# NVIDIA/audio-flamingo

Measured on AMD Instinct MI355X. Metric: audio-sec/s + decoder tokens/s, AF3-7B bf16 train, higher is better.
Workload: dtype bf16; 1 GPU; AF3 (AF-Whisper 32L + Qwen2.5-7B 28L, MLP projector) bf16 train step fwd+bwd+AdamW, 30 s clips, S=1024; micro_batch_per_gpu=8, global_batch=8, seq_len=1024, parallelism=dp1, activation_checkpointing=False

## Files before the change

### audio-flamingo_amd/csrc/common.h

```cpp
#pragma once
#include <hip/hip_runtime.h>
#include <stdint.h>
#include <stdio.h>
#include <stdarg.h>
#include <type_traits>
#include <utility>

typedef __bf16 bf16;
typedef __attribute__((ext_vector_type(2))) __bf16 bf16x2;
typedef __attribute__((ext_vector_type(4))) __bf16 bf16x4;
typedef __attribute__((ext_vector_type(8))) __bf16 bf16x8;
typedef __attribute__((ext_vector_type(2))) float f32x2;
typedef __attribute__((ext_vector_type(4))) float f32x4;
typedef __attribute__((ext_vector_type(16))) float f32x16;

#define AFK_OK 0
#define AFK_ERR_ARG (-1)
#define AFK_ERR_LAUNCH (-2)
#define AFK_ERR_UNSUPPORTED (-3)

int afk_set_error(int code, const char* fmt, ...);
void afk_count(int id);

#define AFK_REQUIRE(cond, ...)                                   \
// ... 80 lines not shown
}

__device__ __forceinline__ float bf2f(bf16 x) { return (float)x; }
__device__ __forceinline__ bf16 f2bf(float x) { return (bf16)x; }
__device__ __forceinline__ float rbf(float x) { return (float)((bf16)x); }
__device__ __forceinline__ float rbf_strict(float x) {
    const bf16 h = (bf16)x;
    return __uint_as_float((uint32_t)__builtin_bit_cast(unsigned short, h) << 16);
}

__device__ __forceinline__ float wave_sum(float v) {
#pragma unroll
    for (int o = 32; o > 0; o >>= 1) v += __shfl_xor(v, o, 64);
    return v;
}
__device__ __forceinline__ float wave_max(float v) {
#pragma unroll
    for (int o = 32; o > 0; o >>= 1) v = fmaxf(v, __shfl_xor(v, o, 64));
    return v;
}

template <int NW>
__device__ __forceinline__ float block_sum(float v, float* scratch) {
    v = wave_sum(v);
    const int lane = threadIdx.x & 63, w = threadIdx.x >> 6;
    __syncthreads();
    if (lane == 0) scratch[w] = v;
    __syncthreads();
    float r = 0.f;
#pragma unroll
    for (int i = 0; i < NW; ++i) r += scratch[i];
    return r;
}
template <int NW>
__device__ __forceinline__ float block_max(float v, float* scratch) {
    v = wave_max(v);
    const int lane = threadIdx.x & 63, w = threadIdx.x >> 6;
    __syncthreads();
    if (lane == 0) scratch[w] = v;
    __syncthreads();
    float r = scratch[0];
#pragma unroll
    for (int i = 1; i < NW; ++i) r = fmaxf(r, scratch[i]);
    return r;
}

__device__ __forceinline__ float sigmoid_f(float x) { return 1.f / (1.f + __expf(-x)); }
__device__ __forceinline__ float gelu_f(float x) { return 0.5f * x * (1.f + erff(x * 0.70710678118654752440f)); }
__device__ __forceinline__ float gelu_grad_f(float x) {
    const float cdf = 0.5f * (1.f + erff(x * 0.70710678118654752440f));
    const float pdf = 0.39894228040143267794f * __expf(-0.5f * x * x);
    return cdf + x * pdf;
}
```

### audio-flamingo_amd/csrc/elementwise.hip

```cpp
#include "common.h"
#include "../../include/afk.h"

namespace {

inline int ew_grid(int64_t n_items, int per_block) {
    int64_t g = afk_cdiv(n_items, per_block);
    if (g > 4096) g = 4096;
    if (g < 1) g = 1;
    return (int)g;
}

__global__ __launch_bounds__(256) void transpose_kernel(const bf16* __restrict__ in0, bf16* __restrict__ out0, int R, int C,
                                                        int Rpad, int64_t ld_in, int64_t ld_out, int nb2,
                                                        int64_t bs1_in, int64_t bs2_in, int64_t bs1_out, int64_t bs2_out,
                                                        int tiles_x, int tiles_y, int64_t ntiles) {
    __shared__ bf16 tile[64][66];
    const int t = threadIdx.x;
    for (int64_t tix = blockIdx.x; tix < ntiles; tix += gridDim.x) {
        const int bx = (int)(tix % tiles_x);
        const int by = (int)((tix / tiles_x) % tiles_y);
        const int b = (int)(tix / ((int64_t)tiles_x * tiles_y));
        const int b1 = b / nb2, b2 = b - b1 * nb2;
        const bf16* in = in0 + b1 * bs1_in + b2 * bs2_in;
        bf16* out = out0 + b1 * bs1_out + b2 * bs2_out;
// ... 94 lines not shown
            const float silu = gf * s;
            og[e] = (bf16)(df * uf * (s * (1.f + gf * (1.f - s))));
            ou[e] = (bf16)(df * silu);
        }
        *(bf16x8*)(dgu + r * 2 * I + c) = og;
        *(bf16x8*)(dgu + r * 2 * I + I + c) = ou;
    }
}

__global__ __launch_bounds__(256) void rope_kernel(bf16* __restrict__ buf, const bf16* __restrict__ cos_t,
                                                   const bf16* __restrict__ sin_t, const int* __restrict__ pos, int64_t rows,
                                                   int S, int ld, int nheads, int D, float sign) {
    const int half = D >> 1, vph = half >> 2;
    const int64_t total = rows * nheads * vph;
    for (int64_t i = (int64_t)blockIdx.x * 256 + threadIdx.x; i < total; i += (int64_t)gridDim.x * 256) {
        const int v = (int)(i % vph);
        const int64_t t = i / vph;
        const int h = (int)(t % nheads);
        const int64_t r = t / nheads;
        const int p = pos ? pos[r] : (int)(r % S);
        bf16* x1p = buf + r * ld + h * D + 4 * v;
        bf16* x2p = x1p + half;
        const bf16x4 x1 = *(const bf16x4*)x1p, x2 = *(const bf16x4*)x2p;
        const bf16x4 c1 = *(const bf16x4*)(cos_t + (int64_t)p * D + 4 * v);
        const bf16x4 s1 = *(const bf16x4*)(sin_t + (int64_t)p * D + 4 * v);
        const bf16x4 c2 = *(const bf16x4*)(cos_t + (int64_t)p * D + half + 4 * v);
        const bf16x4 s2 = *(const bf16x4*)(sin_t + (int64_t)p * D + half + 4 * v);
        bf16x4 o1, o2;
#pragma unroll
        for (int e = 0; e < 4; ++e) {
            const float a = (float)x1[e], b = (float)x2[e];
            o1[e] = (bf16)(rbf_strict(a * (float)c1[e]) + rbf_strict(-sign * b * (float)s1[e]));
            o2[e] = (bf16)(rbf_strict(b * (float)c2[e]) + rbf_strict(sign * a * (float)s2[e]));
        }
        *(bf16x4*)x1p = o1;
        *(bf16x4*)x2p = o2;
    }
}

__global__ __launch_bounds__(256) void add_kernel(const bf16* __restrict__ a, const bf16* __restrict__ b, bf16* __restrict__ o,
                                                  int64_t nvec) {
    for (int64_t i = (int64_t)blockIdx.x * 256 + threadIdx.x; i < nvec; i += (int64_t)gridDim.x * 256) {
        const bf16x8 x = *(const bf16x8*)(a + 8 * i), y = *(const bf16x8*)(b + 8 * i);
        bf16x8 r;
#pragma unroll
        for (int e = 0; e < 8; ++e) r[e] = (bf16)((float)x[e] + (float)y[e]);
        *(bf16x8*)(o + 8 * i) = r;
    }
}

__global__ __launch_bounds__(256) void scale_add_kernel(const bf16* x, bf16* y, int64_t nvec, const float* __restrict__ scale,
                                                        int accumulate) {
    const float a = *scale;
    for (int64_t i = (int64_t)blockIdx.x * 256 + threadIdx.x; i < nvec; i += (int64_t)gridDim.x * 256) {
        const bf16x8 xv = *(const bf16x8*)(x + 8 * i);
        bf16x8 o;
        if (accumulate) {
            const bf16x8 yv = *(const bf16x8*)(y + 8 * i);
#pragma unroll
            for (int e = 0; e < 8; ++e) o[e] = (bf16)((float)yv[e] + a * (float)xv[e]);
        } else {
#pragma unroll
            for (int e = 0; e < 8; ++e) o[e] = (bf16)(a * (float)xv[e]);
        }
        *(bf16x8*)(y + 8 * i) = o;
    }
}

__global__ __launch_bounds__(256) void cast_f32_bf16_kernel(const float* __restrict__ a, bf16* __restrict__ o, int64_t n) {
    for (int64_t i = (int64_t)blockIdx.x * 256 + threadIdx.x; i < n; i += (int64_t)gridDim.x * 256) o[i] = (bf16)a[i];
}

__global__ __launch_bounds__(256) void rowsum_kernel(const bf16* __restrict__ in, int64_t ld, int C, bf16* __restrict__ out,
                                                     int rows, int accumulate) {
    const int lane = threadIdx.x & 63;
    const int row = blockIdx.x * 4 + (threadIdx.x >> 6);
    if (row >= rows) return;
    const bf16* p = in + (int64_t)row * ld;
    float s = 0.f;
    const int nv = C >> 3;
    for (int v = lane; v < nv; v += 64) {
        const bf16x8 t = *(const bf16x8*)(p + 8 * v);
#pragma unroll
        for (int e = 0; e < 8; ++e) s += (float)t[e];
    }
    for (int c = nv * 8 + lane; c < C; c += 64) s += (float)p[c];
    s = wave_sum(s);
    if (lane == 0) out[row] = (bf16)(accumulate ? s + (float)out[row] : s);
}

template <bool FUSED>
__global__ __launch_bounds__(256) void colsum_partial_kernel(const bf16* __restrict__ in, int64_t ld, int64_t rows, int cols,
                                                             float* __restrict__ partial, int rows_per_slice, int* __restrict__ counters,
                                                             bf16* __restrict__ out, int accumulate) {
    __shared__ float red[32][65];
    __shared__ int last_flag;
    const int cl = threadIdx.x & 7, rl = threadIdx.x >> 3;
    const int c0 = blockIdx.x * 64 + cl * 8;
    const int64_t r_begin = (int64_t)blockIdx.y * rows_per_slice;
    const int64_t r_end = min(rows, r_begin + rows_per_slice);
    float acc[8];
#pragma unroll
    for (int e = 0; e < 8; ++e) acc[e] = 0.f;
    if (c0 < cols) {
        for (int64_t r = r_begin + rl; r < r_end; r += 32) {
            const bf16x8 t = *(const bf16x8*)(in + r * ld + c0);
// ... 194 lines not shown
        __syncthreads();
    }
    if (tid == 0) *n_audio = carry;
}

__global__ __launch_bounds__(256) void embed_scatter_fwd_kernel(const int64_t* __restrict__ ids, const int* __restrict__ src,
                                                                const bf16* __restrict__ embed, const bf16* __restrict__ audio,
                                                                bf16* __restrict__ out, int64_t n, int H) {
    const int vpr = H >> 3;
    const int64_t total = n * vpr;
    for (int64_t i = (int64_t)blockIdx.x * 256 + threadIdx.x; i < total; i += (int64_t)gridDim.x * 256) {
        const int v = (int)(i % vpr);
        const int64_t r = i / vpr;
        const int s = src ? src[r] : -1;
        const bf16* p = (s >= 0) ? audio + (int64_t)s * H : embed + ids[r] * H;
        *(bf16x8*)(out + r * H + 8 * v) = *(const bf16x8*)(p + 8 * v);
    }
}

__global__ __launch_bounds__(256) void embed_scatter_bwd_kernel(const int64_t* __restrict__ ids, const int* __restrict__ src,
                                                                const bf16* __restrict__ dout, bf16* __restrict__ d_embed,
                                                                bf16* __restrict__ d_audio, const int* __restrict__ perm, int64_t n, int H) {
    const int vpr = H >> 3;
    const int64_t total = n * vpr;
    for (int64_t i = (int64_t)blockIdx.x * 256 + threadIdx.x; i < total; i += (int64_t)gridDim.x * 256) {
        const int v = (int)(i % vpr);
        const int64_t j = i / vpr;
        const int64_t r = perm ? perm[j] : j;
        const int s = src ? src[r] : -1;
        if (s >= 0) {
            if (d_audio) *(bf16x8*)(d_audio + (int64_t)s * H + 8 * v) = *(const bf16x8*)(dout + r * H + 8 * v);
            continue;
        }
        if (!d_embed) continue;
        const int64_t id = ids[r];
        if (j > 0 && ids[perm[j - 1]] == id) continue;
        float acc[8] = {0.f, 0.f, 0.f, 0.f, 0.f, 0.f, 0.f, 0.f};
        for (int64_t k = j; k < n; ++k) {
            const int64_t rk = perm[k];
            if (ids[rk] != id) break;
            const bf16x8 d = *(const bf16x8*)(dout + rk * H + 8 * v);
#pragma unroll
            for (int e = 0; e < 8; ++e) acc[e] += (float)d[e];
        }
        bf16* p = d_embed + id * H + 8 * v;
        const bf16x8 old = *(const bf16x8*)p;
        bf16x8 o;
#pragma unroll
        for (int e = 0; e < 8; ++e) o[e] = (bf16)((float)old[e] + acc[e]);
        *(bf16x8*)p = o;
    }
}

__device__ __forceinline__ float adamw_elem(float& w, float& mm, float& vv, float gr, float lr, float b1, float b2, float eps, float wd, float bc1,
                                            float bc2_sqrt) {
#pragma clang fp contract(off)
    w = w * (1.f - lr * wd);
    mm = b1 * mm + (1.f - b1) * gr;
    vv = b2 * vv + ((1.f - b2) * gr) * gr;
    const float denom = sqrtf(vv) / bc2_sqrt + eps;
    w = w - (lr / bc1) * (mm / denom);
    return w;
}

__global__ __launch_bounds__(256) void adamw_kernel(float* __restrict__ master, float* __restrict__ m, float* __restrict__ v,
                                                    const bf16* __restrict__ g, bf16* __restrict__ p, int64_t n, float lr,
                                                    float b1, float b2, float eps, float wd, float bc1, float bc2_sqrt,
                                                    float grad_scale, const int* __restrict__ gate, const float* __restrict__ hyper) {
    if (gate != nullptr && *gate == 0) return;
    if (hyper != nullptr) {
        lr = hyper[0];
        bc1 = hyper[1];
        bc2_sqrt = hyper[2];
        grad_scale *= hyper[3];
    }
    const int64_t nv = n >> 2;
    for (int64_t i = (int64_t)blockIdx.x * 256 + threadIdx.x; i < nv; i += (int64_t)gridDim.x * 256) {
        f32x4 w = *(const f32x4*)(master + 4 * i), mm = *(const f32x4*)(m + 4 * i), vv = *(const f32x4*)(v + 4 * i);
        const bf16x4 gg = *(const bf16x4*)(g + 4 * i);
        bf16x4 o;
#pragma unroll
        for (int e = 0; e < 4; ++e) {
            float we = w[e], me = mm[e], ve = vv[e];
            o[e] = (bf16)adamw_elem(we, me, ve, (float)gg[e] * grad_scale, lr, b1, b2, eps, wd, bc1, bc2_sqrt);
            w[e] = we, mm[e] = me, vv[e] = ve;
        }
        *(f32x4*)(master + 4 * i) = w;
        *(f32x4*)(m + 4 * i) = mm;
        *(f32x4*)(v + 4 * i) = vv;
        *(bf16x4*)(p + 4 * i) = o;
    }
    if (blockIdx.x == 0 && threadIdx.x < (n & 3)) {
        const int64_t i = (nv << 2) + threadIdx.x;
        float w = master[i], mm = m[i], vv = v[i];
        adamw_elem(w, mm, vv, (float)g[i] * grad_scale, lr, b1, b2, eps, wd, bc1, bc2_sqrt);
        master[i] = w;
        m[i] = mm;
        v[i] = vv;
        p[i] = (bf16)w;
    }
}


__global__ __launch_bounds__(256) void adamw_t_kernel(float* __restrict__ master, float* __restrict__ m, float* __restrict__ v,
                                                      const bf16* __restrict__ g, bf16* __restrict__ p, bf16* __restrict__ shadow, int N, int K,
                                                      int64_t ld_shadow, float lr, float b1, float b2, float eps, float wd, float bc1,
                                                      float bc2_sqrt, float grad_scale, const int* __restrict__ gate, const float* __restrict__ hyper) {
    if (gate != nullptr && *gate == 0) return;
    if (hyper != nullptr) {
        lr = hyper[0];
        bc1 = hyper[1];
        bc2_sqrt = hyper[2];
        grad_scale *= hyper[3];
    }
    __shared__ bf16 tile[64][66];
    const int t = threadIdx.x;
    const int tiles_x = K >> 6;
    const int64_t ntiles = (int64_t)tiles_x * (N >> 6);
    for (int64_t tix = blockIdx.x; tix < ntiles; tix += gridDim.x) {
        const int n0 = (int)(tix / tiles_x) * 64, k0 = (int)(tix % tiles_x) * 64;
#pragma unroll 1
        for (int j = 0; j < 4; ++j) {
            const int r = (t >> 4) + 16 * j, c4 = (t & 15) * 4;
            const int64_t off = (int64_t)(n0 + r) * K + k0 + c4;
            f32x4 w = *(const f32x4*)(master + off), mm = *(const f32x4*)(m + off), vv = *(const f32x4*)(v + off);
            const bf16x4 gg = *(const bf16x4*)(g + off);
            bf16x4 o;
#pragma unroll
            for (int e = 0; e < 4; ++e) {
                float we = w[e], me = mm[e], ve = vv[e];
                o[e] = (bf16)adamw_elem(we, me, ve, (float)gg[e] * grad_scale, lr, b1, b2, eps, wd, bc1, bc2_sqrt);
                w[e] = we, mm[e] = me, vv[e] = ve;
            }
            *(f32x4*)(master + off) = w;
            *(f32x4*)(m + off) = mm;
            *(f32x4*)(v + off) = vv;
            *(bf16x4*)(p + off) = o;
#pragma unroll
            for (int e = 0; e < 4; ++e) tile[c4 + e][r] = o[e];
        }
        __syncthreads();
#pragma unroll
        for (int j = 0; j < 2; ++j) {
            const int idx = t + 256 * j;
            const int c = idx >> 3, ch = idx & 7;
            bf16x8 o;
#pragma unroll
            for (int e = 0; e < 8; ++e) o[e] = tile[c][ch * 8 + e];
            *(bf16x8*)(shadow + (int64_t)(k0 + c) * ld_shadow + n0 + ch * 8) = o;
        }
        __syncthreads();
    }
}

__device__ __forceinline__ void adamw16_elem(float& w, float& mm, float& vv, float gr, float lr, float omb1, float b2, float omb2, float eps, float wd,
                                             float bc1, float bc2_sqrt) {
#pragma clang fp contract(off)
    w = w - (lr * wd) * w;
    mm = mm + omb1 * (gr - mm);
    vv = b2 * vv + (omb2 * gr) * gr;
    const float denom = sqrtf(vv) / bc2_sqrt + eps;
    w = w - ((lr / bc1) * mm) / denom;
}

__device__ __forceinline__ void adamw16_vec(bf16x8& pp, bf16x8& mm, bf16x8& vv, const bf16x8 gg, float lr, float omb1, float b2, float omb2, float eps,
                                            float wd, float bc1, float bc2_sqrt, float grad_scale) {
#pragma unroll
    for (int e = 0; e < 8; ++e) {
        float we = (float)pp[e], me = (float)mm[e], ve = (float)vv[e];
        adamw16_elem(we, me, ve, (float)gg[e] * grad_scale, lr, omb1, b2, omb2, eps, wd, bc1, bc2_sqrt);
        pp[e] = (bf16)we, mm[e] = (bf16)me, vv[e] = (bf16)ve;
    }
}

__global__ __launch_bounds__(256) void adamw16_kernel(bf16* __restrict__ p, bf16* __restrict__ m, bf16* __restrict__ v, const bf16* __restrict__ g,
                                                      int64_t n, float lr, float omb1, float b2, float omb2, float eps, float wd, float bc1,
                                                      float bc2_sqrt, float grad_scale, const int* __restrict__ gate, const float* __restrict__ hyper) {
    if (gate != nullptr && *gate == 0) return;
    if (hyper != nullptr) {
        lr = hyper[0];
        bc1 = hyper[1];
        bc2_sqrt = hyper[2];
        grad_scale *= hyper[3];
    }
    const int64_t nv = n >> 3;
    for (int64_t i = (int64_t)blockIdx.x * 256 + threadIdx.x; i < nv; i += (int64_t)gridDim.x * 256) {
        bf16x8 pp = *(const bf16x8*)(p + 8 * i), mm = *(const bf16x8*)(m + 8 * i), vv = *(const bf16x8*)(v + 8 * i);
        const bf16x8 gg = *(const bf16x8*)(g + 8 * i);
        adamw16_vec(pp, mm, vv, gg, lr, omb1, b2, omb2, eps, wd, bc1, bc2_sqrt, grad_scale);
        *(bf16x8*)(p + 8 * i) = pp;
        *(bf16x8*)(m + 8 * i) = mm;
        *(bf16x8*)(v + 8 * i) = vv;
    }
    if (blockIdx.x == 0 && threadIdx.x < (n & 7)) {
        const int64_t i = (nv << 3) + threadIdx.x;
        float w = (float)p[i], mm = (float)m[i], vv = (float)v[i];
        adamw16_elem(w, mm, vv, (float)g[i] * grad_scale, lr, omb1, b2, omb2, eps, wd, bc1, bc2_sqrt);
        p[i] = (bf16)w;
        m[i] = (bf16)mm;
        v[i] = (bf16)vv;
    }
}

__global__ __launch_bounds__(256) void adamw16_t_kernel(bf16* __restrict__ p, bf16* __restrict__ m, bf16* __restrict__ v, const bf16* __restrict__ g,
                                                        bf16* __restrict__ shadow, int N, int K, int64_t ld_shadow, float lr, float omb1, float b2,
                                                        float omb2, float eps, float wd, float bc1, float bc2_sqrt, float grad_scale,
                                                        const int* __restrict__ gate, const float* __restrict__ hyper) {
    if (gate != nullptr && *gate == 0) return;
    if (hyper != nullptr) {
        lr = hyper[0];
        bc1 = hyper[1];
        bc2_sqrt = hyper[2];
        grad_scale *= hyper[3];
    }
    __shared__ bf16 tile[64][66];
    const int t = threadIdx.x;
    const int tiles_x = K >> 6;
    const int64_t ntiles = (int64_t)tiles_x * (N >> 6);
    for (int64_t tix = blockIdx.x; tix < ntiles; tix += gridDim.x) {
        const int n0 = (int)(tix / tiles_x) * 64, k0 = (int)(tix % tiles_x) * 64;
#pragma unroll 1
        for (int j = 0; j < 2; ++j) {
            const int r = (t >> 3) + 32 * j, c8 = (t & 7) * 8;
            const int64_t off = (int64_t)(n0 + r) * K + k0 + c8;
            bf16x8 pp = *(const bf16x8*)(p + off), mm = *(const bf16x8*)(m + off), vv = *(const bf16x8*)(v + off);
            const bf16x8 gg = *(const bf16x8*)(g + off);
            adamw16_vec(pp, mm, vv, gg, lr, omb1, b2, omb2, eps, wd, bc1, bc2_sqrt, grad_scale);
            *(bf16x8*)(p + off) = pp;
            *(bf16x8*)(m + off) = mm;
            *(bf16x8*)(v + off) = vv;
#pragma unroll
            for (int e = 0; e < 8; ++e) tile[c8 + e][r] = pp[e];
        }
        __syncthreads();
#pragma unroll
        for (int j = 0; j < 2; ++j) {
            const int idx = t + 256 * j;
            const int c = idx >> 3, ch = idx & 7;
            bf16x8 o;
#pragma unroll
            for (int e = 0; e < 8; ++e) o[e] = tile[c][ch * 8 + e];
            *(bf16x8*)(shadow + (int64_t)(k0 + c) * ld_shadow + n0 + ch * 8) = o;
        }
        __syncthreads();
    }
}

__global__ __launch_bounds__(256) void relu_fwd_kernel(const bf16* __restrict__ x, bf16* __restrict__ y, int64_t nvec) {
    for (int64_t i = (int64_t)blockIdx.x * 256 + threadIdx.x; i < nvec; i += (int64_t)gridDim.x * 256) {
        const bf16x8 v = *(const bf16x8*)(x + 8 * i);
        bf16x8 o;
#pragma unroll
        for (int e = 0; e < 8; ++e) o[e] = (float)v[e] > 0.f ? v[e] : (bf16)0.f;
        *(bf16x8*)(y + 8 * i) = o;
    }
}
__global__ __launch_bounds__(256) void relu_bwd_kernel(const bf16* __restrict__ dy, const bf16* __restrict__ y, bf16* __restrict__ dx,
                                                       int64_t nvec) {
    for (int64_t i = (int64_t)blockIdx.x * 256 + threadIdx.x; i < nvec; i += (int64_t)gridDim.x * 256) {
        const bf16x8 d = *(const bf16x8*)(dy + 8 * i), v = *(const bf16x8*)(y + 8 * i);
        bf16x8 o;
#pragma unroll
        for (int e = 0; e < 8; ++e) o[e] = (float)v[e] > 0.f ? d[e] : (bf16)0.f;
        *(bf16x8*)(dx + 8 * i) = o;
    }
}
__global__ __launch_bounds__(256) void gate_fwd_kernel(const bf16* __restrict__ x, const bf16* __restrict__ h, const bf16* __restrict__ alpha,
                                                       int alpha_vec, const int* __restrict__ gate, bf16* __restrict__ y, int64_t rows,
                                                       int D) {
    const int vpr = D >> 3;
    const int64_t total = rows * vpr;
    for (int64_t i = (int64_t)blockIdx.x * 256 + threadIdx.x; i < total; i += (int64_t)gridDim.x * 256) {
        const int v = (int)(i % vpr);
        const int64_t r = i / vpr;
        const bf16x8 xv = *(const bf16x8*)(x + r * D + 8 * v), hv = *(const bf16x8*)(h + r * D + 8 * v);
        const bool on = gate ? gate[r] != 0 : true;
        bf16x8 o;
#pragma unroll
        for (int e = 0; e < 8; ++e) {
            const float t = rbf(tanhf((float)alpha[alpha_vec ? 8 * v + e : 0]));
            const float g = on ? rbf_strict(t * (float)hv[e]) : 0.f;
            o[e] = (bf16)((float)xv[e] + g);
        }
        *(bf16x8*)(y + r * D + 8 * v) = o;
    }
}
__global__ __launch_bounds__(256) void gate_bwd_kernel(const bf16* __restrict__ dy, const bf16* __restrict__ h, const bf16* __restrict__ alpha,
                                                       int alpha_vec, const int* __restrict__ gate, bf16* __restrict__ dh,
                                                       int64_t rows, int D) {
    const int vpr = D >> 3;
    const int64_t total = rows * vpr;
    for (int64_t i = (int64_t)blockIdx.x * 256 + threadIdx.x; i < total; i += (int64_t)gridDim.x * 256) {
        const int v = (int)(i % vpr);
        const int64_t r = i / vpr;
        const bf16x8 dv = *(const bf16x8*)(dy + r * D + 8 * v), hv = *(const bf16x8*)(h + r * D + 8 * v);
        const bool on = gate ? gate[r] != 0 : true;
        bf16x8 o;
// ... 237 lines not shown
extern "C" int afk_avgpool2_bwd(const void* dy, void* dx, int64_t out_rows, int C, void* stream) {
    AFK_REQUIRE(dy && dx && C % 8 == 0 && out_rows > 0, "afk_avgpool2_bwd: bad args");
    hipLaunchKernelGGL(avgpool2_bwd_kernel, dim3(ew_grid(out_rows * (C / 8), 256)), dim3(256), 0, ST, (const bf16*)dy, (bf16*)dx,
                       out_rows, C);
    AFK_LAUNCH_CHECK("afk_avgpool2_bwd");
    return AFK_OK;
}

extern "C" int afk_placeholder_scan(const int64_t* ids, int64_t n, int64_t audio_id, int* src, int* n_audio, void* stream) {
    AFK_REQUIRE(ids && src && n_audio && n > 0, "afk_placeholder_scan: bad args");
    hipLaunchKernelGGL(placeholder_scan_kernel, dim3(1), dim3(1024), 0, ST, ids, n, audio_id, src, n_audio);
    AFK_LAUNCH_CHECK("afk_placeholder_scan");
    return AFK_OK;
}

extern "C" int afk_embed_scatter_fwd(const int64_t* ids, const int* src, const void* embed, const void* audio, void* out,
                                     int64_t n, int H, void* stream) {
    AFK_REQUIRE(ids && embed && out && n > 0 && H % 8 == 0, "afk_embed_scatter_fwd: bad args");
    AFK_REQUIRE(!src || audio, "afk_embed_scatter_fwd: src without audio rows");
    hipLaunchKernelGGL(embed_scatter_fwd_kernel, dim3(ew_grid(n * (H / 8), 256)), dim3(256), 0, ST, ids, src,
                       (const bf16*)embed, (const bf16*)audio, (bf16*)out, n, H);
    AFK_LAUNCH_CHECK("afk_embed_scatter_fwd");
    return AFK_OK;
}

extern "C" int afk_embed_scatter_bwd(const int64_t* ids, const int* src, const void* dout, void* d_embed, void* d_audio,
                                     const int* perm, int64_t n, int H, void* stream) {
    AFK_REQUIRE(ids && dout && n > 0 && H % 8 == 0, "afk_embed_scatter_bwd: bad args");
    AFK_REQUIRE(perm || !d_embed, "afk_embed_scatter_bwd: d_embed needs perm (rows sorted by token id)");
    hipLaunchKernelGGL(embed_scatter_bwd_kernel, dim3(ew_grid(n * (H / 8), 256)), dim3(256), 0, ST, ids, src,
                       (const bf16*)dout, (bf16*)d_embed, (bf16*)d_audio, perm, n, H);
    AFK_LAUNCH_CHECK("afk_embed_scatter_bwd");
    return AFK_OK;
}

extern "C" int afk_adamw_step(float* master, float* m, float* v, const void* grad, void* param, int64_t n, float lr, float beta1,
                              float beta2, float eps, float weight_decay, int step, float grad_scale, int max_blocks, const int* gate,
                              const float* hyper, void* stream) {
    AFK_REQUIRE(master && m && v && grad && param && n > 0 && step >= 1, "afk_adamw_step: bad args");
    AFK_REQUIRE(((uintptr_t)master % 16 == 0) && ((uintptr_t)m % 16 == 0) && ((uintptr_t)v % 16 == 0) &&
                    ((uintptr_t)grad % 8 == 0) && ((uintptr_t)param % 8 == 0),
                "afk_adamw_step: misaligned buffer");
    const float bc1 = 1.f - powf(beta1, (float)step);
    const float bc2 = 1.f - powf(beta2, (float)step);
    int grid = ew_grid(afk_cdiv(n, 4), 256);
    if (max_blocks > 0 && grid > max_blocks) grid = max_blocks;
    hipLaunchKernelGGL(adamw_kernel, dim3(grid), dim3(256), 0, ST, master, m, v, (const bf16*)grad,
                       (bf16*)param, n, lr, beta1, beta2, eps, weight_decay, bc1, sqrtf(bc2), grad_scale, gate, hyper);
    AFK_LAUNCH_CHECK("afk_adamw_step");
    return AFK_OK;
}


extern "C" int afk_adamw_step_t(float* master, float* m, float* v, const void* grad, void* param, void* shadow, int N, int K, int64_t ld_shadow,
                                float lr, float beta1, float beta2, float eps, float weight_decay, int step, float grad_scale, int max_blocks,
                                const int* gate, const float* hyper, void* stream) {
    AFK_REQUIRE(master && m && v && grad && param && shadow && step >= 1, "afk_adamw_step_t: bad args");
    AFK_REQUIRE(N > 0 && K > 0 && N % 64 == 0 && K % 64 == 0 && ld_shadow >= N && ld_shadow % 8 == 0, "afk_adamw_step_t: N=%d, K=%d must be multiples of 64", N, K);
    AFK_REQUIRE(((uintptr_t)master % 16 == 0) && ((uintptr_t)m % 16 == 0) && ((uintptr_t)v % 16 == 0) && ((uintptr_t)grad % 16 == 0) &&
                    ((uintptr_t)param % 16 == 0) && ((uintptr_t)shadow % 16 == 0),
                "afk_adamw_step_t: misaligned buffer");
    const float bc1 = 1.f - powf(beta1, (float)step);
    const float bc2 = 1.f - powf(beta2, (float)step);
    int64_t grid = (int64_t)(N / 64) * (K / 64);
    if (grid > 16384) grid = 16384;
    if (max_blocks > 0 && grid > max_blocks) grid = max_blocks;
    hipLaunchKernelGGL(adamw_t_kernel, dim3((unsigned)grid), dim3(256), 0, ST, master, m, v, (const bf16*)grad, (bf16*)param, (bf16*)shadow, N, K,
                       ld_shadow, lr, beta1, beta2, eps, weight_decay, bc1, sqrtf(bc2), grad_scale, gate, hyper);
    AFK_LAUNCH_CHECK("afk_adamw_step_t");
    return AFK_OK;
}

extern "C" int afk_adamw16_step(void* m, void* v, const void* grad, void* param, int64_t n, double lr, double beta1, double beta2, double eps,
                                double weight_decay, int step, float grad_scale, int max_blocks, const int* gate, const float* hyper, void* stream) {
    AFK_REQUIRE(m && v && grad && param && n > 0 && step >= 1, "afk_adamw16_step: bad args");
    AFK_REQUIRE(((uintptr_t)m % 16 == 0) && ((uintptr_t)v % 16 == 0) && ((uintptr_t)grad % 16 == 0) && ((uintptr_t)param % 16 == 0),
                "afk_adamw16_step: misaligned buffer");
    const double bc1 = 1.0 - pow(beta1, (double)step), bc2 = 1.0 - pow(beta2, (double)step);
    int grid = ew_grid(afk_cdiv(n, 8), 256);
    if (max_blocks > 0 && grid > max_blocks) grid = max_blocks;
    hipLaunchKernelGGL(adamw16_kernel, dim3(grid), dim3(256), 0, ST, (bf16*)param, (bf16*)m, (bf16*)v, (const bf16*)grad, n, (float)lr,
                       (float)(1.0 - beta1), (float)beta2, (float)(1.0 - beta2), (float)eps, (float)weight_decay, (float)bc1, (float)sqrt(bc2), grad_scale,
                       gate, hyper);
    AFK_LAUNCH_CHECK("afk_adamw16_step");
    return AFK_OK;
}

extern "C" int afk_adamw16_step_t(void* m, void* v, const void* grad, void* param, void* shadow, int N, int K, int64_t ld_shadow, double lr,
                                  double beta1, double beta2, double eps, double weight_decay, int step, float grad_scale, int max_blocks,
                                  const int* gate, const float* hyper, void* stream) {
    AFK_REQUIRE(m && v && grad && param && shadow && step >= 1, "afk_adamw16_step_t: bad args");
    AFK_REQUIRE(N > 0 && K > 0 && N % 64 == 0 && K % 64 == 0 && ld_shadow >= N && ld_shadow % 8 == 0, "afk_adamw16_step_t: N=%d, K=%d must be multiples of 64", N, K);
    AFK_REQUIRE(((uintptr_t)m % 16 == 0) && ((uintptr_t)v % 16 == 0) && ((uintptr_t)grad % 16 == 0) && ((uintptr_t)param % 16 == 0) &&
                    ((uintptr_t)shadow % 16 == 0),
                "afk_adamw16_step_t: misaligned buffer");
    const double bc1 = 1.0 - pow(beta1, (double)step), bc2 = 1.0 - pow(beta2, (double)step);
    int64_t grid = (int64_t)(N / 64) * (K / 64);
    if (grid > 16384) grid = 16384;
    if (max_blocks > 0 && grid > max_blocks) grid = max_blocks;
    hipLaunchKernelGGL(adamw16_t_kernel, dim3((unsigned)grid), dim3(256), 0, ST, (bf16*)param, (bf16*)m, (bf16*)v, (const bf16*)grad, (bf16*)shadow, N, K,
                       ld_shadow, (float)lr, (float)(1.0 - beta1), (float)beta2, (float)(1.0 - beta2), (float)eps, (float)weight_decay, (float)bc1,
                       (float)sqrt(bc2), grad_scale, gate, hyper);
    AFK_LAUNCH_CHECK("afk_adamw16_step_t");
    return AFK_OK;
}

namespace {
constexpr int SUMSQ_BLOCKS = 1024;
__global__ __launch_bounds__(256) void sumsq_partial_kernel(const bf16* __restrict__ x, int64_t n, float* __restrict__ ws) {
    __shared__ float red[4];
    float acc = 0.f;
    const int64_t nv = n >> 3;
    for (int64_t i = (int64_t)blockIdx.x * 256 + threadIdx.x; i < nv; i += (int64_t)gridDim.x * 256) {
        const bf16x8 v = *(const bf16x8*)(x + 8 * i);
#pragma unroll
        for (int e = 0; e < 8; ++e) acc += (float)v[e] * (float)v[e];
    }
    if (blockIdx.x == 0 && threadIdx.x < (n & 7)) {
        const float t = (float)x[(nv << 3) + threadIdx.x];
        acc += t * t;
    }
    acc = block_sum<4>(acc, red);
    if (threadIdx.x == 0) ws[blockIdx.x] = acc;
}
__global__ __launch_bounds__(256) void sumsq_fold_kernel(const float* __restrict__ ws, int nblk, float* __restrict__ acc, const int* __restrict__ gate) {
    __shared__ float red[4];
    float s = 0.f;
    for (int i = threadIdx.x; i < nblk; i += 256) s += ws[i];
    s = block_sum<4>(s, red);
    if (threadIdx.x == 0 && (gate == nullptr || *gate != 0)) acc[0] += s;
}
__global__ void clip_coef_kernel(const float* sumsq, int n, float scale, float max_norm, float* coef, float* norm_out) {
    if (threadIdx.x == 0) {
        float tot = 0.f;
        for (int i = 0; i < n; ++i) tot += sumsq[i];
        const float norm = sqrtf(tot) * scale;
        const float c = max_norm / (norm + 1e-6f);
        coef[0] = c < 1.f ? c : 1.f;
        if (norm_out) norm_out[0] = norm;
    }
}
}

extern "C" int afk_sumsq_workspace_floats(void) { return SUMSQ_BLOCKS; }
extern "C" int afk_sumsq_bf16(const void* x, int64_t n, float* acc, const int* gate, float* workspace, void* stream) {
    AFK_REQUIRE(x && acc && workspace && n > 0, "afk_sumsq_bf16: bad args");
    AFK_REQUIRE(((uintptr_t)x & 15) == 0, "afk_sumsq_bf16: x must be 16-byte aligned");
    int grid = (int)afk_cdiv(afk_cdiv(n, 8), 256);
    if (grid > SUMSQ_BLOCKS) grid = SUMSQ_BLOCKS;
    hipLaunchKernelGGL(sumsq_partial_kernel, dim3(grid), dim3(256), 0, ST, (const bf16*)x, n, workspace);
    hipLaunchKernelGGL(sumsq_fold_kernel, dim3(1), dim3(256), 0, ST, workspace, grid, acc, gate);
    AFK_LAUNCH_CHECK("afk_sumsq_bf16");
    return AFK_OK;
}
extern "C" int afk_clip_coef(const float* sumsq, int n, float scale, float max_norm, float* coef, float* norm_out, void* stream) {
    AFK_REQUIRE(sumsq && coef && n >= 1 && max_norm > 0.f && scale > 0.f, "afk_clip_coef: bad args");
// ... 122 lines not shown
```

Baseline: 639.3 audio-s/s.

## Move transposed AdamW kernels to strip tiling with swizzled LDS and prefetch

```diff
diff --git a/audio-flamingo_amd/csrc/adamw_shadow.hip b/audio-flamingo_amd/csrc/adamw_shadow.hip
--- /dev/null
+++ b/audio-flamingo_amd/csrc/adamw_shadow.hip
@@ -0,0 +1,245 @@
+#include "common.h"
+#include "../../include/afk.h"
+
+namespace {
+
+constexpr int STRIP_R = 64, STRIP_C = 256;
+constexpr int STRIP_LDS_BYTES = STRIP_R * STRIP_C * (int)sizeof(bf16);
+
+__device__ __forceinline__ void strip_geometry(unsigned six, unsigned strips_k, int& n0, int& k0) {
+    const unsigned sn = six / strips_k;
+    n0 = __builtin_amdgcn_readfirstlane((int)sn * STRIP_R);
+    k0 = __builtin_amdgcn_readfirstlane((int)(six - sn * strips_k) * STRIP_C);
+}
+
+__device__ __forceinline__ int64_t uniform64(int64_t x) {
+    const unsigned lo = __builtin_amdgcn_readfirstlane((unsigned)x), hi = __builtin_amdgcn_readfirstlane((unsigned)((uint64_t)x >> 32));
+    return (int64_t)(((uint64_t)hi << 32) | lo);
+}
+__device__ __forceinline__ void make_opaque(int& x) { asm volatile("" : "+v"(x)); }
+
+template <bool FULL>
+__device__ __forceinline__ void strip_store_rows(const bf16 (*tile)[STRIP_R], bf16* __restrict__ out, int64_t ld_shadow, int krows, int t) {
+#pragma unroll
+    for (int it = 0; it < STRIP_C * 8 / 256; ++it) {
+        const int idx = t + 256 * it;
+        const int kk = idx >> 3, ch = idx & 7, f = (kk >> 2) & 31;
+        if (FULL || kk < krows) {
+            bf16x8 o = *(const bf16x8*)&tile[kk][(ch ^ (f >> 2)) * 8];
+            if (f & 1) o = __builtin_shufflevector(o, o, 2, 3, 0, 1, 6, 7, 4, 5);
+            if (f & 2) o = __builtin_shufflevector(o, o, 4, 5, 6, 7, 0, 1, 2, 3);
+            *(bf16x8*)(out + (int64_t)kk * ld_shadow + ch * 8) = o;
+        }
+        if ((it & 3) == 3) __builtin_amdgcn_sched_barrier(0);
+    }
+}
+__device__ __forceinline__ void strip_store_shadow(const bf16 (*tile)[STRIP_R], bf16* __restrict__ out, int64_t ld_shadow, int krows, int t) {
+    if (krows >= STRIP_C)
+        strip_store_rows<true>(tile, out, ld_shadow, krows, t);
+    else
+        strip_store_rows<false>(tile, out, ld_shadow, krows, t);
+}
+__device__ __forceinline__ void strip_put_pair(bf16 (*tile)[STRIP_R], unsigned c4, int n, int t, const bf16x4 r0, const bf16x4 r1) {
+#pragma unroll
+    for (int e = 0; e < 4; ++e) {
+        const bf16x2 pk = {r0[e], r1[e]};
+        *(bf16x2*)&tile[c4 + e][((n >> 1) ^ (t & 31)) * 2] = pk;
+    }
+}
+
+__global__ __launch_bounds__(256) __attribute__((amdgpu_waves_per_eu(8, 8))) void adamw_t_kernel(
+    float* __restrict__ master, float* __restrict__ m, float* __restrict__ v, const bf16* __restrict__ g, bf16* __restrict__ p,
+    bf16* __restrict__ shadow, int N, int K, int64_t ld_shadow, float lr, float b1, float b2, float eps, float wd, float bc1, float bc2_sqrt,
+    float grad_scale, const int* __restrict__ gate, const float* __restrict__ hyper) {
+    if (gate != nullptr && *gate == 0) return;
+    if (hyper != nullptr) {
+        lr = hyper[0];
+        bc1 = hyper[1];
+        bc2_sqrt = hyper[2];
+        grad_scale *= hyper[3];
+    }
+    extern __shared__ __attribute__((aligned(16))) bf16 strip_lds[];
+    bf16(*tile)[STRIP_R] = (bf16(*)[STRIP_R])strip_lds;
+    int t = threadIdx.x;
+    const int rg = __builtin_amdgcn_readfirstlane(t >> 6);
+    const unsigned strips_k = ((unsigned)K + STRIP_C - 1) / STRIP_C;
+    const unsigned nstrips = strips_k * ((unsigned)N / STRIP_R);
+    unsigned six = blockIdx.x;
+    if (six >= nstrips) return;
+    int n0, k0;
+    strip_geometry(six, strips_k, n0, k0);
+    f32x4 w[2], mm[2], vv[2];
+    bf16x4 gg[2];
+    auto row_off = [&](int n0_, int k0_, int jj) { return uniform64((int64_t)(n0_ + 16 * (jj >> 2) + 4 * rg + (jj & 3)) * K + k0_); };
+    auto load_row = [&](int n0_, int k0_, int jj, int b, unsigned c4) {
+        if (k0_ + c4 < (unsigned)K) {
+            const int64_t off = row_off(n0_, k0_, jj);
+            w[b] = *(const f32x4*)(master + off + c4), mm[b] = *(const f32x4*)(m + off + c4), vv[b] = *(const f32x4*)(v + off + c4);
+            gg[b] = *(const bf16x4*)(g + off + c4);
+        }
+    };
+    make_opaque(t);
+    load_row(n0, k0, 0, 0, (t & 63) * 4);
+    load_row(n0, k0, 1, 1, (t & 63) * 4);
+    for (;;) {
+#pragma unroll 1
+        for (int i = 0; i < 4; ++i) {
+            make_opaque(t);
+            const unsigned c4 = (t & 63) * 4;
+            const bool act = k0 + c4 < (unsigned)K;
+            bf16x4 o[2];
+#pragma unroll
+            for (int j = 0; j < 4; ++j) {
+                const int b = j & 1, jj = 4 * i + j;
+                if (act) {
+                    const int64_t off = row_off(n0, k0, jj);
+#pragma unroll
+                    for (int e = 0; e < 4; ++e) {
+                        float we = w[b][e], me = mm[b][e], ve = vv[b][e];
+                        o[b][e] = (bf16)adamw_elem(we, me, ve, (float)gg[b][e] * grad_scale, lr, b1, b2, eps, wd, bc1, bc2_sqrt);
+                        w[b][e] = we, mm[b][e] = me, vv[b][e] = ve;
+                    }
+                    *(f32x4*)(master + off + c4) = w[b];
+                    *(f32x4*)(m + off + c4) = mm[b];
+                    *(f32x4*)(v + off + c4) = vv[b];
+                    *(bf16x4*)(p + off + c4) = o[b];
+                    if (b) strip_put_pair(tile, c4, 16 * i + 4 * rg + j - 1, t, o[0], o[1]);
+                }
+                if (jj + 2 < 16) load_row(n0, k0, jj + 2, b, c4);
+                __builtin_amdgcn_sched_barrier(0);
+            }
+        }
+        __syncthreads();
+        make_opaque(t);
+        const int pn0 = n0, pk0 = k0;
+        six += gridDim.x;
+        const bool more = six < nstrips;
+        if (more) {
+            strip_geometry(six, strips_k, n0, k0);
+            load_row(n0, k0, 0, 0, (t & 63) * 4);
+            load_row(n0, k0, 1, 1, (t & 63) * 4);
+        }
+        __builtin_amdgcn_sched_barrier(0);
+        strip_store_shadow(tile, shadow + (int64_t)pk0 * ld_shadow + pn0, ld_shadow, K - pk0, t);
+        if (!more) break;
+        __syncthreads();
+    }
+}
+
+__global__ __launch_bounds__(256) __attribute__((amdgpu_waves_per_eu(8, 8))) void adamw16_t_kernel(
+    bf16* __restrict__ p, bf16* __restrict__ m, bf16* __restrict__ v, const bf16* __restrict__ g, bf16* __restrict__ shadow, int N, int K,
+    int64_t ld_shadow, float lr, float omb1, float b2, float omb2, float eps, float wd, float bc1, float bc2_sqrt, float grad_scale,
+    const int* __restrict__ gate, const float* __restrict__ hyper) {
+    if (gate != nullptr && *gate == 0) return;
+    if (hyper != nullptr) {
+        lr = hyper[0];
+        bc1 = hyper[1];
+        bc2_sqrt = hyper[2];
+        grad_scale *= hyper[3];
+    }
+    extern __shared__ __attribute__((aligned(16))) bf16 strip_lds[];
+    bf16(*tile)[STRIP_R] = (bf16(*)[STRIP_R])strip_lds;
+    int t = threadIdx.x;
+    const int rg = __builtin_amdgcn_readfirstlane(t >> 6);
+    const unsigned strips_k = ((unsigned)K + STRIP_C - 1) / STRIP_C;
+    const unsigned nstrips = strips_k * ((unsigned)N / STRIP_R);
+    unsigned six = blockIdx.x;
+    if (six >= nstrips) return;
+    int n0, k0;
+    strip_geometry(six, strips_k, n0, k0);
+    bf16x4 pp[2], mm[2], vv[2], gg[2];
+    auto row_off = [&](int n0_, int k0_, int jj) { return uniform64((int64_t)(n0_ + 16 * (jj >> 2) + 4 * rg + (jj & 3)) * K + k0_); };
+    auto load_pair = [&](int n0_, int k0_, int u, unsigned c4) {
+        if (k0_ + c4 < (unsigned)K) {
+#pragma unroll
+            for (int r = 0; r < 2; ++r) {
+                const int64_t off = row_off(n0_, k0_, 2 * u + r);
+                pp[r] = *(const bf16x4*)(p + off + c4), mm[r] = *(const bf16x4*)(m + off + c4), vv[r] = *(const bf16x4*)(v + off + c4);
+                gg[r] = *(const bf16x4*)(g + off + c4);
+            }
+        }
+    };
+    make_opaque(t);
+    load_pair(n0, k0, 0, (t & 63) * 4);
+    for (;;) {
+#pragma unroll 1
+        for (int u = 0; u < 8; ++u) {
+            make_opaque(t);
+            const unsigned c4 = (t & 63) * 4;
+            if (k0 + c4 < (unsigned)K) {
+                bf16x8 p8 = __builtin_shufflevector(pp[0], pp[1], 0, 1, 2, 3, 4, 5, 6, 7);
+                bf16x8 m8 = __builtin_shufflevector(mm[0], mm[1], 0, 1, 2, 3, 4, 5, 6, 7);
+                bf16x8 v8 = __builtin_shufflevector(vv[0], vv[1], 0, 1, 2, 3, 4, 5, 6, 7);
+                const bf16x8 g8 = __builtin_shufflevector(gg[0], gg[1], 0, 1, 2, 3, 4, 5, 6, 7);
+                adamw16_vec(p8, m8, v8, g8, lr, omb1, b2, omb2, eps, wd, bc1, bc2_sqrt, grad_scale);
+                const bf16x4 o0 = __builtin_shufflevector(p8, p8, 0, 1, 2, 3), o1 = __builtin_shufflevector(p8, p8, 4, 5, 6, 7);
+                const int64_t off0 = row_off(n0, k0, 2 * u), off1 = row_off(n0, k0, 2 * u + 1);
+                *(bf16x4*)(p + off0 + c4) = o0;
+                *(bf16x4*)(m + off0 + c4) = __builtin_shufflevector(m8, m8, 0, 1, 2, 3);
+                *(bf16x4*)(v + off0 + c4) = __builtin_shufflevector(v8, v8, 0, 1, 2, 3);
+                *(bf16x4*)(p + off1 + c4) = o1;
+                *(bf16x4*)(m + off1 + c4) = __builtin_shufflevector(m8, m8, 4, 5, 6, 7);
+                *(bf16x4*)(v + off1 + c4) = __builtin_shufflevector(v8, v8, 4, 5, 6, 7);
+                strip_put_pair(tile, c4, 16 * (u >> 1) + 4 * rg + 2 * (u & 1), t, o0, o1);
+            }
+            if (u + 1 < 8) load_pair(n0, k0, u + 1, c4);
+        }
+        __syncthreads();
+        make_opaque(t);
+        const int pn0 = n0, pk0 = k0;
+        six += gridDim.x;
+        const bool more = six < nstrips;
+        if (more) {
+            strip_geometry(six, strips_k, n0, k0);
+            load_pair(n0, k0, 0, (t & 63) * 4);
+        }
+        __builtin_amdgcn_sched_barrier(0);
+        strip_store_shadow(tile, shadow + (int64_t)pk0 * ld_shadow + pn0, ld_shadow, K - pk0, t);
+        if (!more) break;
+        __syncthreads();
+    }
+}
+
+}
+
+#define ST ((hipStream_t)stream)
+
+static int strip_grid(int N, int K, int max_blocks) {
+    int64_t grid = (int64_t)(N / STRIP_R) * afk_cdiv(K, STRIP_C);
+    if (grid > 0x7fffffff) return 0;
+    if (grid > 16384) grid = 16384;
+    if (max_blocks > 0 && grid > max_blocks) grid = max_blocks;
+    return (int)grid;
+}
+
+extern "C" int afk_adamw_step_t(float* master, float* m, float* v, const void* grad, void* param, void* shadow, int N, int K, int64_t ld_shadow,
+                                float lr, float beta1, float beta2, float eps, float weight_decay, int step, float grad_scale, int max_blocks,
+                                const int* gate, const float* hyper, void* stream) {
+    AFK_REQUIRE(master && m && v && grad && param && shadow && step >= 1, "afk_adamw_step_t: bad args");
+    AFK_REQUIRE(N > 0 && K > 0 && N % 64 == 0 && K % 64 == 0 && ld_shadow >= N && ld_shadow % 8 == 0, "afk_adamw_step_t: N=%d, K=%d must be multiples of 64", N, K);
+    AFK_REQUIRE(((uintptr_t)master % 16 == 0) && ((uintptr_t)m % 16 == 0) && ((uintptr_t)v % 16 == 0) && ((uintptr_t)grad % 16 == 0) &&
+                    ((uintptr_t)param % 16 == 0) && ((uintptr_t)shadow % 16 == 0),
+                "afk_adamw_step_t: misaligned buffer");
+    const float bc1 = 1.f - powf(beta1, (float)step);
+    const float bc2 = 1.f - powf(beta2, (float)step);
+    hipLaunchKernelGGL(adamw_t_kernel, dim3((unsigned)strip_grid(N, K, max_blocks)), dim3(256), STRIP_LDS_BYTES, ST, master, m, v, (const bf16*)grad,
+                       (bf16*)param, (bf16*)shadow, N, K, ld_shadow, lr, beta1, beta2, eps, weight_decay, bc1, sqrtf(bc2), grad_scale, gate, hyper);
+    AFK_LAUNCH_CHECK("afk_adamw_step_t");
+    return AFK_OK;
+}
+
+extern "C" int afk_adamw16_step_t(void* m, void* v, const void* grad, void* param, void* shadow, int N, int K, int64_t ld_shadow, double lr,
+                                  double beta1, double beta2, double eps, double weight_decay, int step, float grad_scale, int max_blocks,
+                                  const int* gate, const float* hyper, void* stream) {
+    AFK_REQUIRE(m && v && grad && param && shadow && step >= 1, "afk_adamw16_step_t: bad args");
+    AFK_REQUIRE(N > 0 && K > 0 && N % 64 == 0 && K % 64 == 0 && ld_shadow >= N && ld_shadow % 8 == 0, "afk_adamw16_step_t: N=%d, K=%d must be multiples of 64", N, K);
+    AFK_REQUIRE(((uintptr_t)m % 16 == 0) && ((uintptr_t)v % 16 == 0) && ((uintptr_t)grad % 16 == 0) && ((uintptr_t)param % 16 == 0) &&
+                    ((uintptr_t)shadow % 16 == 0),
+                "afk_adamw16_step_t: misaligned buffer");
+    const double bc1 = 1.0 - pow(beta1, (double)step), bc2 = 1.0 - pow(beta2, (double)step);
+    hipLaunchKernelGGL(adamw16_t_kernel, dim3((unsigned)strip_grid(N, K, max_blocks)), dim3(256), STRIP_LDS_BYTES, ST, (bf16*)param, (bf16*)m, (bf16*)v,
+                       (const bf16*)grad, (bf16*)shadow, N, K, ld_shadow, (float)lr, (float)(1.0 - beta1), (float)beta2, (float)(1.0 - beta2), (float)eps,
+                       (float)weight_decay, (float)bc1, (float)sqrt(bc2), grad_scale, gate, hyper);
+    AFK_LAUNCH_CHECK("afk_adamw16_step_t");
+    return AFK_OK;
+}
diff --git a/audio-flamingo_amd/csrc/common.h b/audio-flamingo_amd/csrc/common.h
--- a/audio-flamingo_amd/csrc/common.h
+++ b/audio-flamingo_amd/csrc/common.h
@@ -156,3 +156,35 @@
     const float pdf = 0.39894228040143267794f * __expf(-0.5f * x * x);
     return cdf + x * pdf;
 }
+
+__device__ __forceinline__ float adamw_elem(float& w, float& mm, float& vv, float gr, float lr, float b1, float b2, float eps, float wd, float bc1,
+                                            float bc2_sqrt) {
+#pragma clang fp contract(off)
+    w = w * (1.f - lr * wd);
+    mm = b1 * mm + (1.f - b1) * gr;
+    vv = b2 * vv + ((1.f - b2) * gr) * gr;
+    const float denom = sqrtf(vv) / bc2_sqrt + eps;
+    w = w - (lr / bc1) * (mm / denom);
+    return w;
+}
+
+
+__device__ __forceinline__ void adamw16_elem(float& w, float& mm, float& vv, float gr, float lr, float omb1, float b2, float omb2, float eps, float wd,
+                                             float bc1, float bc2_sqrt) {
+#pragma clang fp contract(off)
+    w = w - (lr * wd) * w;
+    mm = mm + omb1 * (gr - mm);
+    vv = b2 * vv + (omb2 * gr) * gr;
+    const float denom = sqrtf(vv) / bc2_sqrt + eps;
+    w = w - ((lr / bc1) * mm) / denom;
+}
+
+__device__ __forceinline__ void adamw16_vec(bf16x8& pp, bf16x8& mm, bf16x8& vv, const bf16x8 gg, float lr, float omb1, float b2, float omb2, float eps,
+                                            float wd, float bc1, float bc2_sqrt, float grad_scale) {
+#pragma unroll
+    for (int e = 0; e < 8; ++e) {
+        float we = (float)pp[e], me = (float)mm[e], ve = (float)vv[e];
+        adamw16_elem(we, me, ve, (float)gg[e] * grad_scale, lr, omb1, b2, omb2, eps, wd, bc1, bc2_sqrt);
+        pp[e] = (bf16)we, mm[e] = (bf16)me, vv[e] = (bf16)ve;
+    }
+}
diff --git a/audio-flamingo_amd/csrc/elementwise.hip b/audio-flamingo_amd/csrc/elementwise.hip
--- a/audio-flamingo_amd/csrc/elementwise.hip
+++ b/audio-flamingo_amd/csrc/elementwise.hip
@@ -170,6 +170,7 @@
 __global__ __launch_bounds__(256) void scale_add_kernel(const bf16* x, bf16* y, int64_t nvec, const float* __restrict__ scale,
                                                         int accumulate) {
     const float a = *scale;
+    if (x == y && !accumulate && a == 1.0f) return;
     for (int64_t i = (int64_t)blockIdx.x * 256 + threadIdx.x; i < nvec; i += (int64_t)gridDim.x * 256) {
         const bf16x8 xv = *(const bf16x8*)(x + 8 * i);
         bf16x8 o;
@@ -470,17 +471,6 @@
     }
 }
 
-__device__ __forceinline__ float adamw_elem(float& w, float& mm, float& vv, float gr, float lr, float b1, float b2, float eps, float wd, float bc1,
-                                            float bc2_sqrt) {
-#pragma clang fp contract(off)
-    w = w * (1.f - lr * wd);
-    mm = b1 * mm + (1.f - b1) * gr;
-    vv = b2 * vv + ((1.f - b2) * gr) * gr;
-    const float denom = sqrtf(vv) / bc2_sqrt + eps;
-    w = w - (lr / bc1) * (mm / denom);
-    return w;
-}
-
 __global__ __launch_bounds__(256) void adamw_kernel(float* __restrict__ master, float* __restrict__ m, float* __restrict__ v,
                                                     const bf16* __restrict__ g, bf16* __restrict__ p, int64_t n, float lr,
                                                     float b1, float b2, float eps, float wd, float bc1, float bc2_sqrt,
@@ -520,76 +510,6 @@
 }
 
 
-__global__ __launch_bounds__(256) void adamw_t_kernel(float* __restrict__ master, float* __restrict__ m, float* __restrict__ v,
-                                                      const bf16* __restrict__ g, bf16* __restrict__ p, bf16* __restrict__ shadow, int N, int K,
-                                                      int64_t ld_shadow, float lr, float b1, float b2, float eps, float wd, float bc1,
-                                                      float bc2_sqrt, float grad_scale, const int* __restrict__ gate, const float* __restrict__ hyper) {
-    if (gate != nullptr && *gate == 0) return;
-    if (hyper != nullptr) {
-        lr = hyper[0];
-        bc1 = hyper[1];
-        bc2_sqrt = hyper[2];
-        grad_scale *= hyper[3];
-    }
-    __shared__ bf16 tile[64][66];
-    const int t = threadIdx.x;
-    const int tiles_x = K >> 6;
-    const int64_t ntiles = (int64_t)tiles_x * (N >> 6);
-    for (int64_t tix = blockIdx.x; tix < ntiles; tix += gridDim.x) {
-        const int n0 = (int)(tix / tiles_x) * 64, k0 = (int)(tix % tiles_x) * 64;
-#pragma unroll 1
-        for (int j = 0; j < 4; ++j) {
-            const int r = (t >> 4) + 16 * j, c4 = (t & 15) * 4;
-            const int64_t off = (int64_t)(n0 + r) * K + k0 + c4;
-            f32x4 w = *(const f32x4*)(master + off), mm = *(const f32x4*)(m + off), vv = *(const f32x4*)(v + off);
-            const bf16x4 gg = *(const bf16x4*)(g + off);
-            bf16x4 o;
-#pragma unroll
-            for (int e = 0; e < 4; ++e) {
-                float we = w[e], me = mm[e], ve = vv[e];
-                o[e] = (bf16)adamw_elem(we, me, ve, (float)gg[e] * grad_scale, lr, b1, b2, eps, wd, bc1, bc2_sqrt);
-                w[e] = we, mm[e] = me, vv[e] = ve;
-            }
-            *(f32x4*)(master + off) = w;
-            *(f32x4*)(m + off) = mm;
-            *(f32x4*)(v + off) = vv;
-            *(bf16x4*)(p + off) = o;
-#pragma unroll
-            for (int e = 0; e < 4; ++e) tile[c4 + e][r] = o[e];
-        }
-        __syncthreads();
-#pragma unroll
-        for (int j = 0; j < 2; ++j) {
-            const int idx = t + 256 * j;
-            const int c = idx >> 3, ch = idx & 7;
-            bf16x8 o;
-#pragma unroll
-            for (int e = 0; e < 8; ++e) o[e] = tile[c][ch * 8 + e];
-            *(bf16x8*)(shadow + (int64_t)(k0 + c) * ld_shadow + n0 + ch * 8) = o;
-        }
-        __syncthreads();
-    }
-}
-
-__device__ __forceinline__ void adamw16_elem(float& w, float& mm, float& vv, float gr, float lr, float omb1, float b2, float omb2, float eps, float wd,
-                                             float bc1, float bc2_sqrt) {
-#pragma clang fp contract(off)
-    w = w - (lr * wd) * w;
-    mm = mm + omb1 * (gr - mm);
-    vv = b2 * vv + (omb2 * gr) * gr;
-    const float denom = sqrtf(vv) / bc2_sqrt + eps;
-    w = w - ((lr / bc1) * mm) / denom;
-}
-
-__device__ __forceinline__ void adamw16_vec(bf16x8& pp, bf16x8& mm, bf16x8& vv, const bf16x8 gg, float lr, float omb1, float b2, float omb2, float eps,
-                                            float wd, float bc1, float bc2_sqrt, float grad_scale) {
-#pragma unroll
-    for (int e = 0; e < 8; ++e) {
-        float we = (float)pp[e], me = (float)mm[e], ve = (float)vv[e];
-        adamw16_elem(we, me, ve, (float)gg[e] * grad_scale, lr, omb1, b2, omb2, eps, wd, bc1, bc2_sqrt);
-        pp[e] = (bf16)we, mm[e] = (bf16)me, vv[e] = (bf16)ve;
-    }
-}
 
 __global__ __launch_bounds__(256) void adamw16_kernel(bf16* __restrict__ p, bf16* __restrict__ m, bf16* __restrict__ v, const bf16* __restrict__ g,
                                                       int64_t n, float lr, float omb1, float b2, float omb2, float eps, float wd, float bc1,
@@ -617,50 +537,6 @@
         p[i] = (bf16)w;
         m[i] = (bf16)mm;
         v[i] = (bf16)vv;
-    }
-}
-
-__global__ __launch_bounds__(256) void adamw16_t_kernel(bf16* __restrict__ p, bf16* __restrict__ m, bf16* __restrict__ v, const bf16* __restrict__ g,
-                                                        bf16* __restrict__ shadow, int N, int K, int64_t ld_shadow, float lr, float omb1, float b2,
-                                                        float omb2, float eps, float wd, float bc1, float bc2_sqrt, float grad_scale,
-                                                        const int* __restrict__ gate, const float* __restrict__ hyper) {
-    if (gate != nullptr && *gate == 0) return;
-    if (hyper != nullptr) {
-        lr = hyper[0];
-        bc1 = hyper[1];
-        bc2_sqrt = hyper[2];
-        grad_scale *= hyper[3];
-    }
-    __shared__ bf16 tile[64][66];
-    const int t = threadIdx.x;
-    const int tiles_x = K >> 6;
-    const int64_t ntiles = (int64_t)tiles_x * (N >> 6);
-    for (int64_t tix = blockIdx.x; tix < ntiles; tix += gridDim.x) {
-        const int n0 = (int)(tix / tiles_x) * 64, k0 = (int)(tix % tiles_x) * 64;
-#pragma unroll 1
-        for (int j = 0; j < 2; ++j) {
-            const int r = (t >> 3) + 32 * j, c8 = (t & 7) * 8;
-            const int64_t off = (int64_t)(n0 + r) * K + k0 + c8;
-            bf16x8 pp = *(const bf16x8*)(p + off), mm = *(const bf16x8*)(m + off), vv = *(const bf16x8*)(v + off);
-            const bf16x8 gg = *(const bf16x8*)(g + off);
-            adamw16_vec(pp, mm, vv, gg, lr, omb1, b2, omb2, eps, wd, bc1, bc2_sqrt, grad_scale);
-            *(bf16x8*)(p + off) = pp;
-            *(bf16x8*)(m + off) = mm;
-            *(bf16x8*)(v + off) = vv;
-#pragma unroll
-            for (int e = 0; e < 8; ++e) tile[c8 + e][r] = pp[e];
-        }
-        __syncthreads();
-#pragma unroll
-        for (int j = 0; j < 2; ++j) {
-            const int idx = t + 256 * j;
-            const int c = idx >> 3, ch = idx & 7;
-            bf16x8 o;
-#pragma unroll
-            for (int e = 0; e < 8; ++e) o[e] = tile[c][ch * 8 + e];
-            *(bf16x8*)(shadow + (int64_t)(k0 + c) * ld_shadow + n0 + ch * 8) = o;
-        }
-        __syncthreads();
     }
 }
 
@@ -1004,25 +880,6 @@
 }
 
 
-extern "C" int afk_adamw_step_t(float* master, float* m, float* v, const void* grad, void* param, void* shadow, int N, int K, int64_t ld_shadow,
-                                float lr, float beta1, float beta2, float eps, float weight_decay, int step, float grad_scale, int max_blocks,
-                                const int* gate, const float* hyper, void* stream) {
-    AFK_REQUIRE(master && m && v && grad && param && shadow && step >= 1, "afk_adamw_step_t: bad args");
-    AFK_REQUIRE(N > 0 && K > 0 && N % 64 == 0 && K % 64 == 0 && ld_shadow >= N && ld_shadow % 8 == 0, "afk_adamw_step_t: N=%d, K=%d must be multiples of 64", N, K);
-    AFK_REQUIRE(((uintptr_t)master % 16 == 0) && ((uintptr_t)m % 16 == 0) && ((uintptr_t)v % 16 == 0) && ((uintptr_t)grad % 16 == 0) &&
-                    ((uintptr_t)param % 16 == 0) && ((uintptr_t)shadow % 16 == 0),
-                "afk_adamw_step_t: misaligned buffer");
-    const float bc1 = 1.f - powf(beta1, (float)step);
-    const float bc2 = 1.f - powf(beta2, (float)step);
-    int64_t grid = (int64_t)(N / 64) * (K / 64);
-    if (grid > 16384) grid = 16384;
-    if (max_blocks > 0 && grid > max_blocks) grid = max_blocks;
-    hipLaunchKernelGGL(adamw_t_kernel, dim3((unsigned)grid), dim3(256), 0, ST, master, m, v, (const bf16*)grad, (bf16*)param, (bf16*)shadow, N, K,
-                       ld_shadow, lr, beta1, beta2, eps, weight_decay, bc1, sqrtf(bc2), grad_scale, gate, hyper);
-    AFK_LAUNCH_CHECK("afk_adamw_step_t");
-    return AFK_OK;
-}
-
 extern "C" int afk_adamw16_step(void* m, void* v, const void* grad, void* param, int64_t n, double lr, double beta1, double beta2, double eps,
                                 double weight_decay, int step, float grad_scale, int max_blocks, const int* gate, const float* hyper, void* stream) {
     AFK_REQUIRE(m && v && grad && param && n > 0 && step >= 1, "afk_adamw16_step: bad args");
@@ -1035,25 +892,6 @@
                        (float)(1.0 - beta1), (float)beta2, (float)(1.0 - beta2), (float)eps, (float)weight_decay, (float)bc1, (float)sqrt(bc2), grad_scale,
                        gate, hyper);
     AFK_LAUNCH_CHECK("afk_adamw16_step");
-    return AFK_OK;
-}
-
-extern "C" int afk_adamw16_step_t(void* m, void* v, const void* grad, void* param, void* shadow, int N, int K, int64_t ld_shadow, double lr,
-                                  double beta1, double beta2, double eps, double weight_decay, int step, float grad_scale, int max_blocks,
-                                  const int* gate, const float* hyper, void* stream) {
-    AFK_REQUIRE(m && v && grad && param && shadow && step >= 1, "afk_adamw16_step_t: bad args");
-    AFK_REQUIRE(N > 0 && K > 0 && N % 64 == 0 && K % 64 == 0 && ld_shadow >= N && ld_shadow % 8 == 0, "afk_adamw16_step_t: N=%d, K=%d must be multiples of 64", N, K);
-    AFK_REQUIRE(((uintptr_t)m % 16 == 0) && ((uintptr_t)v % 16 == 0) && ((uintptr_t)grad % 16 == 0) && ((uintptr_t)param % 16 == 0) &&
-                    ((uintptr_t)shadow % 16 == 0),
-                "afk_adamw16_step_t: misaligned buffer");
-    const double bc1 = 1.0 - pow(beta1, (double)step), bc2 = 1.0 - pow(beta2, (double)step);
-    int64_t grid = (int64_t)(N / 64) * (K / 64);
-    if (grid > 16384) grid = 16384;
-    if (max_blocks > 0 && grid > max_blocks) grid = max_blocks;
-    hipLaunchKernelGGL(adamw16_t_kernel, dim3((unsigned)grid), dim3(256), 0, ST, (bf16*)param, (bf16*)m, (bf16*)v, (const bf16*)grad, (bf16*)shadow, N, K,
-                       ld_shadow, (float)lr, (float)(1.0 - beta1), (float)beta2, (float)(1.0 - beta2), (float)eps, (float)weight_decay, (float)bc1,
-                       (float)sqrt(bc2), grad_scale, gate, hyper);
-    AFK_LAUNCH_CHECK("afk_adamw16_step_t");
     return AFK_OK;
 }
 
```

After: 640.3 audio-s/s, median of 6. About the same (+0.2%).
